# supyuxiang/Inference-Time-Scaling-for-Diffusion-Models-beyond-Scaling-Denoising-Steps

Measured on NVIDIA B200. Metric: candidate images/sec (T=1000 NFE, verifier incl.), higher is better.
Workload: dtype bf16/fp16 operands, fp32 accumulate

## Files before the change

inference-time-scaling-for-diffusion-models-beyond-scaling-denoising-steps_b200/csrc/conv_persist_sm100.cu:

```cuda
#include "tapgemm.cuh"
#include "sm100_ptx.cuh"

namespace its {

constexpr int P_THREADS = 352;
constexpr int P_EPI_THREADS = 256;
constexpr int PANEL_COLS = 64;
constexpr int PANEL_BYTES = BM * PANEL_COLS * 2;

template <int BN, int STAGES, int MT, int KS, bool TM = false>
struct PersistSmem {
  static constexpr int B_BYTES = BN * BK * 2;
  static constexpr int STAGE_BYTES = KS * (MT * A_BYTES + B_BYTES);
  static constexpr int STAGING_OFF = STAGES * STAGE_BYTES;
  static constexpr int RED_OFF = STAGING_OFF + 2 * PANEL_BYTES;
  static constexpr int RED_BYTES = 2 * 8 * 16 * 8;
  static constexpr int BAR_OFF = RED_OFF + RED_BYTES;
  static constexpr int NBARS = 2 * STAGES + 8;
  static constexpr int TOTAL = BAR_OFF + NBARS * 8 + 16;
  static constexpr int TMEM_COLS = (2 * MT * BN <= 128) ? 128 : (2 * MT * BN <= 256) ? 256 : 512;
  static_assert(2 * MT * BN <= 512, "TMEM holds two accumulator sets");
  static_assert(!TM || (BN == 128 && MT == 2 && KS == 1), "transposed mode: 128 channels x 256 pixels");
};

struct TileCoord {
  int phase, n0, tx, ty, tb;
};

__device__ __forceinline__ TileCoord decode_tile(const TapGemmParams& p, int tile, int tiles_m, int tiles_n,
                                                  int bn, int mt_per_tile) {
  TileCoord c;
  const int tpp = tiles_m * tiles_n;
  c.phase = tile / tpp;
  const int r = tile - c.phase * tpp;
  const int nt = r / tiles_m;
  const int mt = r - nt * tiles_m;
  c.n0 = nt * bn;
  const int ty_tiles = p.tiles_y / mt_per_tile;
  c.tx = mt % p.tiles_x;
  c.ty = (mt / p.tiles_x) % ty_tiles;
  c.tb = mt / (p.tiles_x * ty_tiles);
  return c;
}

struct WorkItem {
  int tile, split;
};
__device__ __forceinline__ WorkItem decode_item(int w, int total_tiles, int S) {
  WorkItem it;
  if (S == 1) {
    it.tile = w;
    it.split = 0;
  } else {
    const int npart = total_tiles * (S - 1);
    if (w < npart) {
      it.tile = w / (S - 1);
      it.split = w - it.tile * (S - 1);
    } else {
      it.tile = w - npart;
      it.split = S - 1;
    }
  }
  return it;
}

template <bool H>
__device__ __forceinline__ void tm_stage_column(const uint32_t* v, float alpha, float bvs, uint32_t sbuf_addr, int half,
                                                uint32_t chunk, uint32_t col_byte, float& s, float& qq) {
#pragma unroll
  for (int i = 0; i < 64; ++i) {
    const uint32_t prow = (uint32_t)(half * 64 + i);
    const float f = fmaf(__uint_as_float(v[i]), alpha, bvs);
    unsigned short hb;
    float r;
    if (H) {
      const __half hh = __float2half_rn(f);
      r = __half2float(hh);
      hb = __half_as_ushort(hh);
    } else {
      const __nv_bfloat16 h = __float2bfloat16_rn(f);
      r = __bfloat162float(h);
      hb = __bfloat16_as_ushort(h);
    }
    s += r;
    qq = fmaf(r, r, qq);
// ... 14 lines not shown
    const uint32_t dst = row_addr + (uint32_t)(((half * 4 + g) ^ (row & 7)) << 4);
    const uint4 u = *reinterpret_cast<const uint4*>(&pk);
    asm volatile("st.shared.v4.b32 [%0], {%1, %2, %3, %4};" ::"r"(dst), "r"(u.x), "r"(u.y), "r"(u.z), "r"(u.w)
                 : "memory");
  }
}

template <bool H>
__device__ __forceinline__ void column_pair_sums(uint32_t sbuf_addr, int r8, int cp, float& s, float& qq) {
#pragma unroll
  for (int i = 0; i < 16; ++i) {
    const int r = r8 * 16 + i;
    const uint32_t a = sbuf_addr + (uint32_t)r * 128u + (uint32_t)((((cp >> 2) ^ (r & 7)) << 4) | ((cp & 3) << 2));
    uint32_t wv;
    asm volatile("ld.shared.b32 %0, [%1];" : "=r"(wv) : "r"(a));
    float x0, x1;
    decode2_fmt(wv, H, x0, x1);
    s += x0 + x1;
    qq = fmaf(x0, x0, qq);
    qq = fmaf(x1, x1, qq);
  }
}

__device__ __forceinline__ void gn_peer_rendezvous(unsigned* counter, unsigned peers) {
  __threadfence();
  const unsigned old = atomicAdd(counter, 1u);
  const unsigned target = (old / peers + 1u) * peers;
  if (old + 1u != target) {
    unsigned cur = old;
    for (uint32_t spin = 0; spin < (1u << 24); ++spin) {
      asm volatile("ld.acquire.gpu.global.u32 %0, [%1];" : "=r"(cur) : "l"(counter) : "memory");
      if ((int)(cur - target) >= 0) break;
      __nanosleep(20);
    }
    if ((int)(cur - target) < 0) __trap();
  }
  __threadfence();
}

__device__ __forceinline__ void gn_tile_stats(float2* table, const float2* stats, int et, int pairs, int ngt, int g0,
                                              int img0, int n_img, int parts, int nchunk, int cg4, double n, float eps) {
  int T = P_EPI_THREADS / pairs;
  if (T > 32) T = 32;
  const int pr = et / T, l = et - pr * T;
  const int il = pr / ngt, gl = pr - il * ngt;
  const long long bi = img0 + il;
  const bool active = pr < pairs && bi < n_img;
  double s = 0.0, q = 0.0;
  if (active) {
    const float2* base = stats + bi * parts * nchunk + (g0 + gl) * cg4;
    const int E = parts * cg4;
// ... 92 lines not shown
    tma_prefetch_desc(&tmB);
    tma_prefetch_desc(&tmOut);
    if constexpr (GN) tma_prefetch_desc(&tmGn);
  }
  if (warp == 1) {
    asm volatile("tcgen05.alloc.cta_group::1.sync.aligned.shared::cta.b32 [%0], %1;" ::"r"(smem_u32(tmem_slot)),
                 "r"((uint32_t)L::TMEM_COLS)
                 : "memory");
    asm volatile("tcgen05.relinquish_alloc_permit.cta_group::1.sync.aligned;" ::: "memory");
  }
  tcgen05_fence_before();
  __syncthreads();
  tcgen05_fence_after();
  const uint32_t tmem_base = *tmem_slot;
  asm volatile("griddepcontrol.launch_dependents;" ::: "memory");
  if (warp != 0) asm volatile("griddepcontrol.wait;" ::: "memory");
  if (dbg != nullptr && threadIdx.x == 0) dbg[2] = clock64();

  if (warp == 0) {
    uint32_t npre = 0;
    auto produce = [&](const bool pre) {
      uint32_t it = 0;
      for (int w = blockIdx.x; w < total_items; w += gridDim.x) {
        const WorkItem wi = decode_item(w, total_tiles, S);
        const TileCoord c = decode_tile(p, wi.tile, tiles_m, tiles_n, BN, MT);
        const DevPhase& ph = p.phase[c.phase];
        const int kb0 = (ph.nkb * wi.split) / S, kb1 = (ph.nkb * (wi.split + 1)) / S;
        const int wb = (p.w_batch_stride != 0) ? c.tb * p.bb : 0;
        int g = 0;
        for (int t = 0; t < ph.ntaps && g < kb1; ++t) {
          const int si = ph.src[t];
          const DevSrc& s = p.src[si];
          const int ncb = s.C / BK;
          if (g + ncb <= kb0) { g += ncb; continue; }
          const CUtensorMap* tm = (si == 0) ? &tmA0 : (si == 1) ? &tmA1 : &tmA2;
          const int cx = c.tx * p.bw * s.stride + ph.dx[t];
          const int cy = c.ty * (p.bh * MT) * s.stride + ph.dy[t];
          const int cb_img = s.bcast ? 0 : c.tb * p.bb;
          for (int cb = 0; cb < ncb; cb += KS, g += KS) {
            if (g < kb0 || g >= kb1) continue;
            if (pre && it >= (uint32_t)STAGES) { npre = it; return; }
            const uint32_t stage = it % STAGES;
            const uint32_t parity = (it / STAGES) & 1u;
            if (!pre) mbar_wait(&empty_bar[stage], parity ^ 1u);
            if (elect_one_sync()) {
              uint8_t* a_dst = smem + stage * L::STAGE_BYTES;
              uint8_t* b_dst = a_dst + KS * MT * A_BYTES;
// ... 2 lines not shown
#pragma unroll
                for (int u = 0; u < KS; ++u)
                  tma_load_3d(b_dst + u * L::B_BYTES, &tmB, &full_bar[stage], ph.w_k0 + (g + u) * BK, c.n0, wb);
              }
              if (!pre) {
#pragma unroll
                for (int u = 0; u < KS; ++u)
                  tma_load_4d(a_dst + u * MT * A_BYTES, tm, &full_bar[stage], (cb + u) * BK, cx, cy, cb_img);
              }
            }
            __syncwarp();
            ++it;
          }
        }
      }
      if (pre) npre = it;
    };
    if (p.w_batch_stride == 0) produce(true);
    asm volatile("griddepcontrol.wait;" ::: "memory");
    produce(false);
  } else if (warp == 1) {
    uint32_t it = 0, j = 0;
    for (int w = blockIdx.x; w < total_items; w += gridDim.x, ++j) {
      const WorkItem wi = decode_item(w, total_tiles, S);
      const DevPhase& ph = p.phase[wi.tile / (tiles_m * tiles_n)];
      const int nkb_phase = ph.nkb;
      const int kb0 = (nkb_phase * wi.split) / S;
      const int nkb = (nkb_phase * (wi.split + 1)) / S - kb0;
      const uint32_t idesc_a = make_idesc(BN, ph.fp16_first != 0), idesc_b = make_idesc(BN, ph.fp16_first == 0);
      const int ksw = ph.kb_switch - kb0;
      const uint32_t buf = j & 1u;
      mbar_wait(&tempty_bar[buf], ((j >> 1) & 1u) ^ 1u);
      tcgen05_fence_after();
      const uint32_t d_tmem = tmem_base + buf * (MT * BN);
      for (int kb = 0; kb < nkb; kb += KS, ++it) {
        const uint32_t stage = it % STAGES;
        const uint32_t parity = (it / STAGES) & 1u;
        const uint32_t idesc = kb < ksw ? idesc_a : idesc_b;
        mbar_wait(&full_bar[stage], parity);
        tcgen05_fence_after();
        if (elect_one_sync()) {
          const uint32_t a_addr = smem_u32(smem + stage * L::STAGE_BYTES);
          const uint32_t b_addr = a_addr + KS * MT * A_BYTES;
          if constexpr (TM) {
            const uint64_t wdesc = make_smem_desc(b_addr), xdesc = make_smem_desc(a_addr);
            const uint32_t idesc_t = (idesc & ~(0x3Fu << 17)) | ((uint32_t)(256 >> 3) << 17);
#pragma unroll
// ... 16 lines not shown
          if (kb + KS >= nkb) umma_commit(&tfull_bar[buf]);
        }
        __syncwarp();
      }
    }
  } else if (warp < 10) {
    const int q = warp & 3;
    const int half = (warp - 2) >> 2;
    const int row = q * 32 + lane;
    const int et = (warp - 2) * 32 + lane;
    const int rpi = BM / p.bb;
    const int rb = row / rpi;
    const int nsb_img = 8 / p.bb;
    const int tiles_img = p.tiles_x * p.tiles_y;
    const int cp = et & 31, r8 = et >> 5;
    const int st_ch = et & 15, st_ib = et >> 4;
    float2* prev_dst = nullptr;
    constexpr bool fuse_gn = GN;
    const bool gn_silu = p.gn_silu != 0;
    const int gn_cg = fuse_gn ? p.Cout / p.gn_groups : 4;
    const float2* stats2 = reinterpret_cast<const float2*>(p.stats);
    uint32_t j = 0, pc = 0;
    for (int w = blockIdx.x; w < total_items; w += gridDim.x, ++j) {
      const WorkItem wi = decode_item(w, total_tiles, S);
      const TileCoord c = decode_tile(p, wi.tile, tiles_m, tiles_n, BN, MT);
      const uint32_t buf = j & 1u;
      constexpr int NPANEL = BN / PANEL_COLS;
      if (S > 1) {
        int* flags = reinterpret_cast<int*>(p.ws);
        float* parts = p.ws + p.ws_flag_words;
        if (wi.split < S - 1) {
          mbar_wait(&tfull_bar[buf], (j >> 1) & 1u);
          tcgen05_fence_after();
          float* wsrow = parts + ((long long)(wi.tile * (S - 1) + wi.split) * BM + row) * BN + half * 32;
#pragma unroll 1
          for (int pn = 0; pn < NPANEL; ++pn) {
            uint32_t v[32];
            tmem_ld32_nowait(tmem_base + ((uint32_t)(q * 32) << 16) + buf * (MT * BN) +
                                 (uint32_t)(pn * PANEL_COLS + half * 32), v);
            tmem_wait_ld();
            float4* dst = reinterpret_cast<float4*>(wsrow + pn * PANEL_COLS);
#pragma unroll
            for (int i = 0; i < 8; ++i)
              __stcg(dst + i, make_float4(__uint_as_float(v[4 * i]), __uint_as_float(v[4 * i + 1]),
                                          __uint_as_float(v[4 * i + 2]), __uint_as_float(v[4 * i + 3])));
          }
          tcgen05_fence_before();
          mbar_arrive(&tempty_bar[buf]);
          __threadfence();
          named_bar_sync(1, P_EPI_THREADS);
          if (et == 0) {
            int* f = flags + wi.tile * (S - 1) + wi.split;
            asm volatile("st.release.gpu.global.s32 [%0], %1;" ::"l"(f), "r"(1) : "memory");
          }
          continue;
        }
        if (et == 0) {
          for (int sp = 0; sp < S - 1; ++sp) {
            int* f = flags + wi.tile * (S - 1) + sp;
            int seen = 0;
            for (uint32_t spin = 0; spin < (1u << 24); ++spin) {
              asm volatile("ld.acquire.gpu.global.s32 %0, [%1];" : "=r"(seen) : "l"(f) : "memory");
              if (seen != 0) break;
              __nanosleep(64);
            }
            if (seen == 0) __trap();
            *f = 0;
          }
        }
        named_bar_sync(1, P_EPI_THREADS);
      }
      if constexpr (TM) {
        const int cglob = c.n0 + row;
        const int bimg = c.tb;
        float bvs = p.bias ? __ldg(p.bias + cglob) : 0.f;
        if (p.vec) bvs += __ldg(p.vec + (long long)bimg * p.vec_stride + cglob);
        if (p.vec2) bvs += __ldg(p.vec2 + (long long)bimg * p.vec2_stride + cglob);
        mbar_wait(&tfull_bar[buf], (j >> 1) & 1u);
        tcgen05_fence_after();
        if (dbg != nullptr && et == 0 && j < 8) dbg[8 + j] = clock64();
        const int pn = q >> 1;
        const uint32_t cc = (uint32_t)((q & 1) * 32 + lane);
#pragma unroll 1
        for (int m = 0; m < 2; ++m) {
          const uint32_t P = pc + 2 * m + pn;
          const uint32_t sb = P & 1u;
          uint8_t* sbuf = staging + sb * PANEL_BYTES;
          uint32_t v[64];
          const uint32_t taddr = tmem_base + ((uint32_t)(q * 32) << 16) + buf * (MT * BN) +
                                 (uint32_t)(m * 128 + half * 64);
          tmem_ld32_nowait(taddr, v);
          tmem_ld32_nowait(taddr + 32, v + 32);
          mbar_wait(&pempty_bar[sb], ((P >> 1) & 1u) ^ 1u);
// ... 6 lines not shown
          const uint32_t col_byte = (cc & 7u) * 2u;
          const uint32_t chunk = cc >> 3;
          tm_stage_column<F16>(v, p.alpha, bvs, smem_u32(sbuf), half, chunk, col_byte, s, qq);
          fence_proxy_async_smem();
          mbar_arrive(&pfull_bar[sb]);
          if (p.stats != nullptr) {
            s += __shfl_xor_sync(0xffffffffu, s, 1);
            qq += __shfl_xor_sync(0xffffffffu, qq, 1);
            s += __shfl_xor_sync(0xffffffffu, s, 2);
            qq += __shfl_xor_sync(0xffffffffu, qq, 2);
            if ((lane & 3) == 0) {
              const int ty = c.ty * MT + m;
              const int part = ((c.phase * tiles_img + ty * p.tiles_x + c.tx) << 1) + half;
              reinterpret_cast<float2*>(p.stats)[((long long)bimg * p.stats_parts + part) * (p.Cout >> 2) + (cglob >> 2)] =
                  make_float2(s, qq);
            }
          }
        }
        pc += 4;
        if constexpr (GN) {
          if (p.gn_peers > 1) {
            named_bar_sync(1, P_EPI_THREADS);
            if (et == 0)
              gn_peer_rendezvous(reinterpret_cast<unsigned*>(p.gn_sync) + c.tb * tiles_n + c.n0 / BN, (unsigned)p.gn_peers);
          } else {
            __threadfence();
          }
          named_bar_sync(1, P_EPI_THREADS);
          const int ngt = BN / gn_cg, g0 = c.n0 / gn_cg;
          gn_tile_stats(red, stats2, et, ngt, ngt, g0, bimg, p.B, p.stats_parts, p.Cout >> 2, gn_cg >> 2,
                        (double)gn_cg * (double)(p.Hm * p.Wm), p.gn_eps);
          named_bar_sync(1, P_EPI_THREADS);
          const float2 mr = red[cglob / gn_cg - g0];
          const float sc = mr.y * __ldg(p.gn_gamma + cglob);
          const float gA = p.alpha * sc;
          const float gB = fmaf(bvs, sc, __ldg(p.gn_beta + cglob) - mr.x * sc);
#pragma unroll 1
          for (int m = 0; m < 2; ++m) {
            const uint32_t P = pc + 2 * m + pn;
            const uint32_t sb = P & 1u;
            uint8_t* sbuf = staging + sb * PANEL_BYTES;
            uint32_t v[64];
            const uint32_t taddr = tmem_base + ((uint32_t)(q * 32) << 16) + buf * (MT * BN) +
                                   (uint32_t)(m * 128 + half * 64);
            tmem_ld32_nowait(taddr, v);
            tmem_ld32_nowait(taddr + 32, v + 32);
            mbar_wait(&pempty_bar[sb], ((P >> 1) & 1u) ^ 1u);
            tmem_wait_ld();
            if (m == 1) {
              tcgen05_fence_before();
              mbar_arrive(&tempty_bar[buf]);
            }
            tm_stage_column_gn(v, gA, gB, gn_silu, smem_u32(sbuf), half, cc >> 3, (cc & 7u) * 2u);
            fence_proxy_async_smem();
            mbar_arrive(&pfull_bar[sb]);
          }
          pc += 4;
          named_bar_sync(1, P_EPI_THREADS);
        }
        if (dbg != nullptr && et == 0 && j < 8) dbg[24 + j] = clock64();
        continue;
      }
      int b = c.tb * p.bb + rb;
      if (b >= p.B) b = p.B - 1;
      const float* vrow = p.vec ? p.vec + (long long)b * p.vec_stride : nullptr;
      const float* vrow2 = p.vec2 ? p.vec2 + (long long)b * p.vec2_stride : nullptr;
#pragma unroll 1
      for (int pi = 0; pi < MT * NPANEL; ++pi, ++pc) {
        const int m = pi / NPANEL, pn = pi - m * NPANEL;
        const int n = c.n0 + pn * PANEL_COLS;
        const int nc = n + half * 32;
        const int ty = c.ty * MT + m;
        const uint32_t sb = pc & 1u, spar = (pc >> 1) & 1u;
        uint8_t* sbuf = staging + sb * PANEL_BYTES;
        float bv[32];
#pragma unroll
        for (int i = 0; i < 32; ++i) bv[i] = 0.f;
        if (p.bias) {
#pragma unroll
          for (int i = 0; i < 8; ++i) {
            const float4 t4 = __ldg(reinterpret_cast<const float4*>(p.bias + nc) + i);
            bv[4 * i] = t4.x; bv[4 * i + 1] = t4.y; bv[4 * i + 2] = t4.z; bv[4 * i + 3] = t4.w;
          }
        }
        if (vrow) {
#pragma unroll
          for (int i = 0; i < 8; ++i) {
            const float4 t4 = __ldg(reinterpret_cast<const float4*>(vrow + nc) + i);
            bv[4 * i] += t4.x; bv[4 * i + 1] += t4.y; bv[4 * i + 2] += t4.z; bv[4 * i + 3] += t4.w;
          }
        }
        if (vrow2) {
#pragma unroll
          for (int i = 0; i < 8; ++i) {
            const float4 t4 = __ldg(reinterpret_cast<const float4*>(vrow2 + nc) + i);
            bv[4 * i] += t4.x; bv[4 * i + 1] += t4.y; bv[4 * i + 2] += t4.z; bv[4 * i + 3] += t4.w;
          }
        }
        if (pi == 0) {
          mbar_wait(&tfull_bar[buf], (j >> 1) & 1u);
          tcgen05_fence_after();
          if (dbg != nullptr && et == 0 && j < 8) dbg[8 + j] = clock64();
        }
        uint32_t v[32];
        const uint32_t taddr = tmem_base + ((uint32_t)(q * 32) << 16) + buf * (MT * BN) +
                               (uint32_t)(m * BN + pn * PANEL_COLS + half * 32);
        tmem_ld32_nowait(taddr, v);
        mbar_wait(&pempty_bar[sb], spar ^ 1u);
        tmem_wait_ld();
        if (pi == MT * NPANEL - 1 && !fuse_gn) {
          tcgen05_fence_before();
          mbar_arrive(&tempty_bar[buf]);
        }
        if (S > 1) {
          const float* prow = p.ws + p.ws_flag_words +
                              ((long long)(wi.tile * (S - 1)) * BM + row) * BN + pn * PANEL_COLS + half * 32;
          float acc[32];
          for (int sp = 0; sp < S - 1; ++sp) {
            const float4* src = reinterpret_cast<const float4*>(prow + (long long)sp * BM * BN);
#pragma unroll
            for (int i = 0; i < 8; ++i) {
              const float4 t4 = __ldcg(src + i);
              if (sp == 0) {
                acc[4 * i] = t4.x; acc[4 * i + 1] = t4.y; acc[4 * i + 2] = t4.z; acc[4 * i + 3] = t4.w;
              } else {
                acc[4 * i] += t4.x; acc[4 * i + 1] += t4.y; acc[4 * i + 2] += t4.z; acc[4 * i + 3] += t4.w;
              }
            }
          }
#pragma unroll
          for (int i = 0; i < 32; ++i) v[i] = __float_as_uint(acc[i] + __uint_as_float(v[i]));
        }
        const uint32_t row_addr = smem_u32(sbuf) + (uint32_t)row * 128u;
        stage_row32<F16>(v, p.alpha, bv, row_addr, half, row);
        fence_proxy_async_smem();
        mbar_arrive(&pfull_bar[sb]);
        if (p.stats != nullptr && p.bb > 8) {
          mbar_wait(&pfull_bar[sb], spar);
          for (int idx = et; idx < p.bb * 16; idx += P_EPI_THREADS) {
            const int ib = idx >> 4, ch = idx & 15;
            const int bi = c.tb * p.bb + ib;
            if (bi >= p.B) continue;
            float s = 0.f, qq = 0.f;
            for (int r = ib * rpi; r < (ib + 1) * rpi; ++r) {
              const uint32_t a = smem_u32(sbuf) + (uint32_t)r * 128u +
                                 (uint32_t)((((ch >> 1) ^ (r & 7)) << 4) | ((ch & 1) << 3));
              uint32_t w0, w1;
              asm volatile("ld.shared.v2.b32 {%0, %1}, [%2];" : "=r"(w0), "=r"(w1) : "r"(a));
              float x0, x1, x2, x3;
              decode2_fmt(w0, F16, x0, x1);
              decode2_fmt(w1, F16, x2, x3);
              s += (x0 + x1) + (x2 + x3);
              qq = fmaf(x0, x0, qq); qq = fmaf(x1, x1, qq); qq = fmaf(x2, x2, qq); qq = fmaf(x3, x3, qq);
            }
// ... 22 lines not shown
          if (et < 16 * p.bb && bi < p.B) {
            const int part = (p.bb == 1) ? c.phase * tiles_img + ty * p.tiles_x + c.tx : c.phase;
            prev_dst = reinterpret_cast<float2*>(p.stats) +
                       ((long long)bi * p.stats_parts + part) * (p.Cout >> 2) + (n >> 2) + st_ch;
          }
        }
      }
      if constexpr (GN) {
        named_bar_sync(1, P_EPI_THREADS);
        if (prev_dst != nullptr) {
          const float2* rd = red + ((pc + 1) & 1u) * 128;
          float S1 = 0.f, Q1 = 0.f;
          for (int k = 0; k < nsb_img; ++k) {
            const float2 t2 = rd[(st_ib * nsb_img + k) * 16 + st_ch];
            S1 += t2.x;
            Q1 += t2.y;
          }
          *prev_dst = make_float2(S1, Q1);
          prev_dst = nullptr;
        }
        if (p.gn_peers > 1) {
          named_bar_sync(1, P_EPI_THREADS);
          if (et == 0)
            gn_peer_rendezvous(reinterpret_cast<unsigned*>(p.gn_sync) + c.tb * tiles_n + c.n0 / BN, (unsigned)p.gn_peers);
        } else {
          __threadfence();
        }
        named_bar_sync(1, P_EPI_THREADS);
        const int NG = BN / gn_cg, g0 = c.n0 / gn_cg;
        gn_tile_stats(red, stats2, et, p.bb * NG, NG, g0, c.tb * p.bb, p.B, p.stats_parts, p.Cout >> 2, gn_cg >> 2,
                      (double)gn_cg * (double)(p.Hm * p.Wm), p.gn_eps);
        named_bar_sync(1, P_EPI_THREADS);
#pragma unroll 1
        for (int pi = 0; pi < MT * NPANEL; ++pi, ++pc) {
          const int m = pi / NPANEL, pn = pi - m * NPANEL;
          const int nc = c.n0 + pn * PANEL_COLS + half * 32;
          const uint32_t sb = pc & 1u, spar = (pc >> 1) & 1u;
          uint8_t* sbuf = staging + sb * PANEL_BYTES;
          uint32_t v[32];
          const uint32_t taddr = tmem_base + ((uint32_t)(q * 32) << 16) + buf * (MT * BN) +
                                 (uint32_t)(m * BN + pn * PANEL_COLS + half * 32);
          tmem_ld32_nowait(taddr, v);
          mbar_wait(&pempty_bar[sb], spar ^ 1u);
          tmem_wait_ld();
          if (pi == MT * NPANEL - 1) {
            tcgen05_fence_before();
            mbar_arrive(&tempty_bar[buf]);
          }
          const float* prow = p.ws + p.ws_flag_words +
                              ((long long)(wi.tile * (S - 1)) * BM + row) * BN + pn * PANEL_COLS + half * 32;
          const uint32_t row_addr = smem_u32(sbuf) + (uint32_t)row * 128u;
#pragma unroll
          for (int k8 = 0; k8 < 4; ++k8) {
            float f[8];
#pragma unroll
            for (int h4 = 0; h4 < 2; ++h4) {
              const int k = 2 * k8 + h4;
              float x[4] = {__uint_as_float(v[4 * k]), __uint_as_float(v[4 * k + 1]), __uint_as_float(v[4 * k + 2]),
                            __uint_as_float(v[4 * k + 3])};
              if (S > 1) {
                float4 acc = __ldcg(reinterpret_cast<const float4*>(prow) + k);
                for (int sp = 1; sp < S - 1; ++sp) {
                  const float4 t4 = __ldcg(reinterpret_cast<const float4*>(prow + (long long)sp * BM * BN) + k);
                  acc.x += t4.x; acc.y += t4.y; acc.z += t4.z; acc.w += t4.w;
                }
                x[0] = acc.x + x[0]; x[1] = acc.y + x[1]; x[2] = acc.z + x[2]; x[3] = acc.w + x[3];
              }
              float add[4] = {0.f, 0.f, 0.f, 0.f};
              if (p.bias) {
                const float4 t4 = __ldg(reinterpret_cast<const float4*>(p.bias + nc) + k);
                add[0] = t4.x; add[1] = t4.y; add[2] = t4.z; add[3] = t4.w;
              }
              if (vrow) {
                const float4 t4 = __ldg(reinterpret_cast<const float4*>(vrow + nc) + k);
                add[0] += t4.x; add[1] += t4.y; add[2] += t4.z; add[3] += t4.w;
              }
              if (vrow2) {
                const float4 t4 = __ldg(reinterpret_cast<const float4*>(vrow2 + nc) + k);
                add[0] += t4.x; add[1] += t4.y; add[2] += t4.z; add[3] += t4.w;
              }
              const float2 mr = red[rb * NG + (nc + 4 * k) / gn_cg - g0];
              const float4 g4 = __ldg(reinterpret_cast<const float4*>(p.gn_gamma + nc) + k);
              const float4 b4 = __ldg(reinterpret_cast<const float4*>(p.gn_beta + nc) + k);
              const float gg[4] = {g4.x, g4.y, g4.z, g4.w}, bt[4] = {b4.x, b4.y, b4.z, b4.w};
#pragma unroll
              for (int jj = 0; jj < 4; ++jj) {
                const float sc = mr.y * gg[jj];
                f[4 * h4 + jj] = gn_act(x[jj], p.alpha * sc, fmaf(add[jj], sc, bt[jj] - mr.x * sc), gn_silu);
              }
            }
// ... 8 lines not shown
        }
        named_bar_sync(1, P_EPI_THREADS);
      }
      if (dbg != nullptr && et == 0 && j < 8) dbg[24 + j] = clock64();
    }
    if (p.stats != nullptr) {
      named_bar_sync(1, P_EPI_THREADS);
      if (prev_dst != nullptr) {
        const float2* rd = red + ((pc + 1) & 1u) * 128;
        float S = 0.f, Q = 0.f;
        for (int k = 0; k < nsb_img; ++k) {
          const float2 t2 = rd[(st_ib * nsb_img + k) * 16 + st_ch];
          S += t2.x;
          Q += t2.y;
        }
        *prev_dst = make_float2(S, Q);
      }
    }
  } else if (warp == 10) {
    if (lane == 0) {
      uint32_t pc = 0;
      constexpr int NPANEL = BN / PANEL_COLS;
      for (int w = blockIdx.x; w < total_items; w += gridDim.x) {
        const WorkItem wi = decode_item(w, total_tiles, S);
        if (wi.split < S - 1) continue;
        const TileCoord c = decode_tile(p, wi.tile, tiles_m, tiles_n, BN, MT);
        const DevPhase& ph = p.phase[c.phase];
        constexpr int npass = GN ? 2 : 1;
        for (int pass = 0; pass < npass; ++pass) {
          for (int pi = 0; pi < MT * NPANEL; ++pi, ++pc) {
            const int m = pi / NPANEL, pn = pi - m * NPANEL;
            const int n = c.n0 + pn * PANEL_COLS;
            const int ty = c.ty * MT + m;
            const uint32_t sb = pc & 1u, spar = (pc >> 1) & 1u;
            const uint8_t* sbuf = staging + sb * PANEL_BYTES;
            mbar_wait(&pfull_bar[sb], spar);
            if (pass == 0 && p.gn_only) {
              mbar_arrive(&pempty_bar[sb]);
              continue;
            }
            if (pass == 1)
              tma_store_3d(&tmGn, sbuf, n, c.tx * p.bw, c.tb * p.bb * p.Hm + ty * p.bh);
            else if (p.out_scale == 1)
              tma_store_3d(&tmOut, sbuf, n, c.tx * p.bw, c.tb * p.bb * p.Hm + ty * p.bh);
            else
              tma_store_5d(&tmOut, sbuf, n, ph.px, c.tx * p.bw, ph.py, c.tb * p.bb * p.Hm + ty * p.bh);
            bulk_commit_group();
            bulk_wait_group_read<0>();
            mbar_arrive(&pempty_bar[sb]);
          }
        }
      }
      bulk_wait_group<0>();
// ... 60 lines not shown
bool tapgemm_persist_eligible(const its_conv_desc* d, const TapGemmParams& p) {
  if (p.out_fp32 || p.out_nchw || p.res != nullptr) return false;
  if (p.w_batch_stride != 0 && (p.bb != 1 || p.splits > 1)) return false;
  if (p.Cout % 64 != 0 || p.out_c_pitch % 8 != 0) return false;
  const int bn = persist_bn(d, p);
  if (!(bn == 64 || bn == 128 || bn == 192 || bn == 256) || p.Cout % bn != 0) return false;
  if (p.bw * p.bh * p.bb != BM || p.Wm % p.bw != 0 || p.Hm % p.bh != 0) return false;
  if (p.bb > 1 && p.bh != p.Hm) return false;
  return true;
}

template <int BN, int STAGES, int MT, int KS, bool TM, bool F16, bool GN>
static int launch_persist_fmt(const TapGemmParams& p, const CUtensorMap* tmA, const CUtensorMap& tmB,
                              const CUtensorMap& tmOut, const CUtensorMap& tmGn, cudaStream_t stream) {
  using L = PersistSmem<BN, STAGES, MT, KS, TM>;
  static_assert(L::TOTAL <= 227 * 1024, "shared memory budget");
  auto kern = tapgemm_persist_kernel<BN, STAGES, MT, KS, TM, F16, GN>;
  static PerDeviceBytes configured;
  if (configured.need(L::TOTAL))
    ITS_CHECK_CUDA(cudaFuncSetAttribute(kern, cudaFuncAttributeMaxDynamicSharedMemorySize, L::TOTAL));
  const int tiles = p.tiles_x * (p.tiles_y / MT) * p.tiles_b * (p.Cout / BN) * p.nphases * p.splits;
  const int sms = device_sm_count();
  cudaLaunchConfig_t cfg = {};
  cfg.gridDim = dim3(tiles < sms ? tiles : sms, 1, 1);
  cfg.blockDim = dim3(P_THREADS, 1, 1);
  cfg.dynamicSmemBytes = L::TOTAL;
  cfg.stream = stream;
  cudaLaunchAttribute attr[1];
  attr[0].id = cudaLaunchAttributeProgrammaticStreamSerialization;
  attr[0].val.programmaticStreamSerializationAllowed = 1;
  cfg.attrs = attr;
  cfg.numAttrs = pdl_enabled(1) ? 1 : 0;
  ITS_CHECK_CUDA(cudaLaunchKernelEx(&cfg, kern, p, tmA[0], tmA[1], tmA[2], tmB, tmOut, tmGn));
  return ITS_OK;
}

template <int BN, int STAGES, int MT, int KS, bool TM = false>
static int launch_persist(const TapGemmParams& p, const CUtensorMap* tmA, const CUtensorMap& tmB,
                          const CUtensorMap& tmOut, const CUtensorMap& tmGn, cudaStream_t stream) {
  if (p.gn_out != nullptr) {
    if (p.out_fp16) return launch_persist_fmt<BN, STAGES, MT, KS, TM, true, true>(p, tmA, tmB, tmOut, tmGn, stream);
    return launch_persist_fmt<BN, STAGES, MT, KS, TM, false, true>(p, tmA, tmB, tmOut, tmGn, stream);
  }
  if (p.out_fp16) return launch_persist_fmt<BN, STAGES, MT, KS, TM, true, false>(p, tmA, tmB, tmOut, tmGn, stream);
  return launch_persist_fmt<BN, STAGES, MT, KS, TM, false, false>(p, tmA, tmB, tmOut, tmGn, stream);
}

int tapgemm_launch_persist(const its_conv_desc* d, const TapGemmParams& p, cudaStream_t stream) {
  const int bn = persist_bn(d, p);
  ITS_REQUIRE(tapgemm_persist_eligible(d, p), "its_conv_igemm: layer not eligible for the persistent kernel");
  ITS_REQUIRE(p.w_pitch % 8 == 0 && (reinterpret_cast<uintptr_t>(p.w) & 15) == 0, "its_conv_igemm: weight alignment");
  ITS_REQUIRE((reinterpret_cast<uintptr_t>(p.out) & 15) == 0, "its_conv_igemm: output pointer alignment");
  if (p.stats != nullptr)
    ITS_REQUIRE(p.stats_parts == tapgemm_stats_parts(d, p), "its_conv_igemm: stats_parts=%d, the tiling writes %d",
                p.stats_parts, tapgemm_stats_parts(d, p));
  const PersistCfg cfg = persist_cfg(d, p);
  const int mt = cfg.mt;
  TapGemmParams pp = p;
  if (p.splits > 1) {
    const long long tiles = (long long)p.tiles_x * p.tiles_y * p.tiles_b * (p.Cout / bn) * p.nphases;
    const long long nflag = ((tiles * (p.splits - 1) + 63) / 64) * 64;
    const long long need = nflag + tiles * (p.splits - 1) * BM * bn;
    ITS_REQUIRE(d->ws != nullptr && d->ws_elems >= need,
                "its_conv_igemm: persistent split-K workspace has %lld floats, %lld needed (must be zero-initialised)",
                (long long)d->ws_elems, need);
    for (int f = 0; f < p.nphases; ++f)
      ITS_REQUIRE(p.splits <= p.phase[f].nkb, "its_conv_igemm: splits=%d exceeds the %d k-blocks of phase %d", p.splits, p.phase[f].nkb, f);
    pp.ws_flag_words = (int)nflag;
  }
  if (p.gn_out != nullptr) {
    const int words = tapgemm_gn_sync_words(d, p);
    ITS_REQUIRE(words >= 0, "its_conv_igemm: this layer's GroupNorm cannot be fused into its epilogue "
                "(its_conv_gn_sync_words() < 0): Cout=%d groups=%d bn=%d", p.Cout, p.gn_groups, bn);
    ITS_REQUIRE(p.stats != nullptr, "its_conv_igemm: the fused GroupNorm epilogue needs the statistics array");
    ITS_REQUIRE(p.gn_gamma != nullptr && p.gn_beta != nullptr, "its_conv_igemm: gn_gamma / gn_beta");
    ITS_REQUIRE(words == 0 || p.gn_sync != nullptr, "its_conv_igemm: gn_sync needs %d zero-initialised ints", words);
    ITS_REQUIRE(p.gn_c_pitch >= p.Cout && p.gn_c_pitch % 8 == 0 && (reinterpret_cast<uintptr_t>(p.gn_out) & 15) == 0,
                "its_conv_igemm: gn_out pitch / alignment");
    pp.gn_sync_words = words;
    pp.gn_peers = p.tiles_x * (p.tiles_y / mt);
  }
  CUtensorMap tmA[ITS_MAX_SRC], tmB, tmOut, tmGn;
  int rc = tapgemm_encode_operand_maps(p, bn, tmA, &tmB, mt);
  if (rc != ITS_OK) return rc;
  const cuuint64_t pitch_b = (cuuint64_t)p.out_c_pitch * 2;
  if (p.out_scale == 1) {
    const cuuint64_t dims[3] = {(cuuint64_t)p.Cout, (cuuint64_t)p.Wm, (cuuint64_t)p.B * p.Hm};
    const cuuint64_t strides[2] = {pitch_b, pitch_b * p.Wout};
    const cuuint32_t box[3] = {(cuuint32_t)PANEL_COLS, (cuuint32_t)p.bw, (cuuint32_t)(p.bh * p.bb)};
    const cuuint32_t estr[3] = {1, 1, 1};
    rc = encode_bf16_map(&tmOut, 3, p.out, dims, strides, box, estr, "output");
// ... 43 lines not shown
```

inference-time-scaling-for-diffusion-models-beyond-scaling-denoising-steps_b200/csrc/tapgemm.cuh:

```cuda
#pragma once
#include "its_common.cuh"
#include <cuda.h>

namespace its {

struct DevSrc {
  const __nv_bfloat16* ptr;
  int c_pitch, C, H, W, stride, bcast, fp16;
};

struct DevPhase {
  int ntaps, w_k0, py, px;
  int nkb;
  int fp16_first;
  int kb_switch;
  int8_t src[ITS_MAX_TAPS], dy[ITS_MAX_TAPS], dx[ITS_MAX_TAPS];
};

struct TapGemmParams {
  DevSrc src[ITS_MAX_SRC];
  DevPhase phase[ITS_MAX_PHASES];
  int nsrc, nphases;
  int B, Hm, Wm;
  const __nv_bfloat16* w;
  int w_pitch;
  long long w_batch_stride;
  int Cout;
  void* out;
  int out_fp32, Hout, Wout, out_scale, out_c_pitch;
  const float* bias;
  const float* vec;
  int vec_stride;
  const float* vec2;
  int vec2_stride;
  const __nv_bfloat16* res;
  int res_c_pitch;
  float alpha;
  int out_nchw;
  int splits;
  float* ws;
  int ws_flag_words;
  long long* dbg;
  float* stats;
  int stats_parts;
  int out_fp16;
  int res_fp16;
  void* gn_out;
  int gn_c_pitch;
  const float* gn_gamma;
  const float* gn_beta;
  int gn_groups;
  float gn_eps;
  int gn_silu, gn_only;
  int* gn_sync;
  int gn_sync_words;
  int gn_peers;
  int bw, bh, bb, tiles_x, tiles_y, tiles_b;
};

int tapgemm_build_params(const its_conv_desc* d, TapGemmParams* p, bool need_k64);
int tapgemm_launch_ref(const TapGemmParams& p, cudaStream_t stream);
int tapgemm_launch_sm100(const its_conv_desc* d, const TapGemmParams& p, cudaStream_t stream);
bool tapgemm_persist_eligible(const its_conv_desc* d, const TapGemmParams& p);
int tapgemm_launch_persist(const its_conv_desc* d, const TapGemmParams& p, cudaStream_t stream);
// ... 11 lines not shown
```

inference-time-scaling-for-diffusion-models-beyond-scaling-denoising-steps_b200/engine.py:

```python
from __future__ import annotations

import ctypes as C
import math
from typing import List, Optional, Sequence, Tuple

import torch

from . import _lib
from ._lib import ConvDesc

BF16 = torch.bfloat16
FP16 = torch.float16
import os as _os
FP16_GN = _os.environ.get("ITS_FP16_GN", "1") != "0"


def _ptr(t: Optional[torch.Tensor]) -> Optional[int]:
    return None if t is None else t.data_ptr()


def pack_conv_weight(w: torch.Tensor) -> torch.Tensor:
    return w.detach().float().permute(0, 2, 3, 1).reshape(w.shape[0], -1)


# ... 90 lines not shown
        return tiles_m, bn

    DESIGN_BATCH = 64

    def _splits_for(self, B, Hm, Wm, cout, nphases, nkb_min, per_image_w) -> int:
        tiles_m, bn = self._tiles(self.DESIGN_BATCH, Hm, Wm, cout, per_image_w)
        ctas = tiles_m * -(-cout // bn) * nphases
        if ctas >= 96:
            return 1
        s = min(148 // ctas, nkb_min // 4, 16)
        return max(1, s)

    @staticmethod
    def _box(Hm: int, Wm: int) -> Tuple[int, int, int]:
        bw = min(Wm, 128)
        bh = min(Hm, 128 // bw)
        return bw, bh, 128 // (bw * bh)

    def _tiles_at(self, B: int, Hm: int, Wm: int) -> int:
        bw, bh, bb = self._box(Hm, Wm)
        return -(-Wm // bw) * -(-Hm // bh) * -(-B // bb)

    _T_KB = {256: 290.0, 192: 250.0, 128: 215.0, 64: 175.0}
    _T_SPLIT2 = 5000.0

    def _fusion_pays(self, Hm, Wm, cout, nkb) -> bool:
        bw, bh, bb = self._box(Hm, Wm)
        return bb == 1 and cout == 128 and Hm * Wm >= 1024 and nkb >= 36

    _SPLIT_BNS = tuple(int(x) for x in _os.environ.get("ITS_SPLIT_BNS", "64").split(","))

    def _persist_plan(self, Hm, Wm, cout, nphases, nkb, group_width: int = 0) -> Tuple[int, int]:
        bw, bh, bb = self._box(Hm, Wm)
        tiles_y = -(-Hm // bh)
        tiles_m = self._tiles_at(self.DESIGN_BATCH, Hm, Wm)
        best = None
        for bn in (256, 192, 128, 64):
            if cout % bn or (group_width and bn % group_width):
                continue
            tiles = tiles_m * (cout // bn) * nphases
            two_rows = bn <= 128 and bb == 1 and tiles_y % 2 == 0
            for S in (1, 2):
                if S > 1 and (bn not in self._SPLIT_BNS or nkb < 16 or tiles * S > self.sm_count or two_rows):
                    break
                if two_rows:
                    rounds = -(-(tiles // 2) // self.sm_count)
                    t = rounds * nkb * 410.0
                else:
                    rounds = -(-(tiles * S) // self.sm_count)
                    t = rounds * -(-nkb // S) * self._T_KB[bn]
                if S > 1:
                    t += self._T_SPLIT2
                if best is None or t < best[0] - 1e-9:
                    best = (t, bn, S)
        if best is None:
            return 0, 0
        return best[1], best[2]

    def conv(self, srcs, phases, Hm, Wm, w, cout, *, out=None, out_scale=1, bias=None, vec=None,
             vec_off=0, vec2=None, vec2_off=0, res=None, alpha=1.0, out_fp32=False, w_batch_stride=0,
             w_pitch=None, B=None, out_shape=None, out_nchw=False, want_stats=True, out_dtype=None,
             fuse_gn=None, gn_only=False) -> torch.Tensor:
        B = self.n_img if B is None else B
        d = ConvDesc()
        d.nsrc = len(srcs)
        for i, (t, c_used, c_off, stride, bcast) in enumerate(srcs):
            s = d.src[i]
            s.ptr, s.c_pitch, s.c_off, s.C = t.data_ptr(), t.shape[-1], c_off, c_used
            s.H, s.W, s.stride, s.bcast = t.shape[1], t.shape[2], stride, int(bcast)
            s.fp16 = int(t.dtype == FP16)
        d.nphases = len(phases)
        flops = 0
        for i, (taps, w_k0, py, px) in enumerate(phases):
            ph = d.phase[i]
            ph.ntaps, ph.w_k0, ph.py, ph.px = len(taps), w_k0, py, px
# ... 39 lines not shown
            bn, splits = 0, 0
            if want_fuse:
                bn, splits = self._persist_plan(Hm, Wm, cout, len(phases), nkb_plan, cout // fuse_gn[0].num_groups)
            if bn == 0:
                want_fuse = False
                bn, splits = self._persist_plan(Hm, Wm, cout, len(phases), nkb_plan)
        if persistent:
            if can_fold:
                k_used = sum(srcs[si][1] for si, _, _ in phases[0][0])
                w = torch.cat([w[:, :k_used].float(), torch.eye(cout, device=w.device)], 1)
                i = d.nsrc
                sN = d.src[i]
                sN.ptr, sN.c_pitch, sN.c_off, sN.C = res.data_ptr(), res.shape[-1], 0, cout
                sN.H, sN.W, sN.stride, sN.bcast = res.shape[1], res.shape[2], 1, 0
                sN.fp16 = int(res.dtype == FP16)
                d.nsrc = i + 1
                ph = d.phase[0]
                ph.src[ph.ntaps], ph.dy[ph.ntaps], ph.dx[ph.ntaps] = i, 0, 0
                ph.ntaps += 1
                d.w_pitch = w.shape[-1]
            d.bn = bn
            if splits > 1:
                tiles = self._tiles_at(B, Hm, Wm) * (cout // bn) * len(phases)
                nflag = -(-(tiles * (splits - 1)) // 64) * 64
                need = nflag + tiles * (splits - 1) * 128 * bn
                if self.ws_persist is None or self.ws_persist.numel() < need:
                    self.ws_persist = torch.zeros(need, dtype=torch.float32, device=self.dev)
                    self.keep.append(self.ws_persist)
                d.splits, d.ws, d.ws_elems = splits, self.ws_persist.data_ptr(), self.ws_persist.numel()
            if want_stats:
                parts = self.L.its_conv_stats_parts(C.byref(d))
                st = self._new((B, parts, cout // 4, 2), torch.float32)
                d.stats, d.stats_parts = st.data_ptr(), parts
                self.stats_of[out.data_ptr()] = (st, parts)
            if want_fuse:
                gnm, gn_silu = fuse_gn
                d.gn_groups = gnm.num_groups
                words = self.L.its_conv_gn_sync_words(C.byref(d))
                if words < 0:
                    d.gn_groups = 0
                else:
                    gn_out = self._new((B, Hout, Wout, cout), FP16)
                    gamma, beta = self._hold(gnm.weight, torch.float32), self._hold(gnm.bias, torch.float32)
                    d.gn_out, d.gn_c_pitch = gn_out.data_ptr(), cout
                    d.gn_gamma, d.gn_beta, d.gn_eps = gamma.data_ptr(), beta.data_ptr(), float(gnm.eps)
                    d.gn_silu, d.gn_only = int(gn_silu), int(bool(gn_only))
                    if words > 0:
                        sync = torch.zeros(words, dtype=torch.int32, device=self.dev)
# ... 410 lines not shown
```

Before: 36.67.

## Replace serial split-K fixup with symmetric reduce-scatter across split peers

Split-K in the persistent conv kernel used to make every non-final split write its full partial tile to a workspace and flag it, while the last split waited and summed everything. Now each split writes only the column strips owned by its peers, meets them at a counter-based rendezvous, and then reduces and runs the epilogue for its own strip, so reduction and epilogue work are spread across all splits. The planner now considers S in {2,4,8} with a byte-based exchange cost model, and the grid is rounded to a multiple of S. The risk is deadlock if split peers are not co-resident, which the grid rounding is meant to prevent. It also adds rendezvous latency on every split tile.

```diff
diff --git a/inference-time-scaling-for-diffusion-models-beyond-scaling-denoising-steps_b200/csrc/conv_persist_sm100.cu b/inference-time-scaling-for-diffusion-models-beyond-scaling-denoising-steps_b200/csrc/conv_persist_sm100.cu
--- a/inference-time-scaling-for-diffusion-models-beyond-scaling-denoising-steps_b200/csrc/conv_persist_sm100.cu
+++ b/inference-time-scaling-for-diffusion-models-beyond-scaling-denoising-steps_b200/csrc/conv_persist_sm100.cu
@@ -46,21 +46,10 @@
 struct WorkItem {
   int tile, split;
 };
-__device__ __forceinline__ WorkItem decode_item(int w, int total_tiles, int S) {
+__device__ __forceinline__ WorkItem decode_item(int w, int S) {
   WorkItem it;
-  if (S == 1) {
-    it.tile = w;
-    it.split = 0;
-  } else {
-    const int npart = total_tiles * (S - 1);
-    if (w < npart) {
-      it.tile = w / (S - 1);
-      it.split = w - it.tile * (S - 1);
-    } else {
-      it.tile = w - npart;
-      it.split = S - 1;
-    }
-  }
+  it.tile = w / S;
+  it.split = w - it.tile * S;
   return it;
 }
 
@@ -121,11 +110,11 @@
   }
 }
 
-__device__ __forceinline__ void gn_peer_rendezvous(unsigned* counter, unsigned peers) {
+__device__ __forceinline__ void peer_rendezvous(unsigned* counter, unsigned quantum, unsigned step) {
   __threadfence();
-  const unsigned old = atomicAdd(counter, 1u);
-  const unsigned target = (old / peers + 1u) * peers;
-  if (old + 1u != target) {
+  const unsigned old = atomicAdd(counter, step);
+  const unsigned target = (old / quantum + 1u) * quantum;
+  if (old + step != target) {
     unsigned cur = old;
     for (uint32_t spin = 0; spin < (1u << 24); ++spin) {
       asm volatile("ld.acquire.gpu.global.u32 %0, [%1];" : "=r"(cur) : "l"(counter) : "memory");
@@ -264,7 +253,7 @@
     auto produce = [&](const bool pre) {
       uint32_t it = 0;
       for (int w = blockIdx.x; w < total_items; w += gridDim.x) {
-        const WorkItem wi = decode_item(w, total_tiles, S);
+        const WorkItem wi = decode_item(w, S);
         const TileCoord c = decode_tile(p, wi.tile, tiles_m, tiles_n, BN, MT);
         const DevPhase& ph = p.phase[c.phase];
         const int kb0 = (ph.nkb * wi.split) / S, kb1 = (ph.nkb * (wi.split + 1)) / S;
@@ -313,7 +302,7 @@
   } else if (warp == 1) {
     uint32_t it = 0, j = 0;
     for (int w = blockIdx.x; w < total_items; w += gridDim.x, ++j) {
-      const WorkItem wi = decode_item(w, total_tiles, S);
+      const WorkItem wi = decode_item(w, S);
       const DevPhase& ph = p.phase[wi.tile / (tiles_m * tiles_n)];
       const int nkb_phase = ph.nkb;
       const int kb0 = (nkb_phase * wi.split) / S;
@@ -376,53 +365,38 @@
     const float2* stats2 = reinterpret_cast<const float2*>(p.stats);
     uint32_t j = 0, pc = 0;
     for (int w = blockIdx.x; w < total_items; w += gridDim.x, ++j) {
-      const WorkItem wi = decode_item(w, total_tiles, S);
+      const WorkItem wi = decode_item(w, S);
       const TileCoord c = decode_tile(p, wi.tile, tiles_m, tiles_n, BN, MT);
       const uint32_t buf = j & 1u;
       constexpr int NPANEL = BN / PANEL_COLS;
+      const int nps = NPANEL / S;
+      const int pi0 = (S > 1) ? wi.split * nps : 0;
+      const int pi1 = (S > 1) ? pi0 + nps : MT * NPANEL;
+      const float* xown = nullptr;
       if (S > 1) {
-        int* flags = reinterpret_cast<int*>(p.ws);
-        float* parts = p.ws + p.ws_flag_words;
-        if (wi.split < S - 1) {
-          mbar_wait(&tfull_bar[buf], (j >> 1) & 1u);
-          tcgen05_fence_after();
-          float* wsrow = parts + ((long long)(wi.tile * (S - 1) + wi.split) * BM + row) * BN + half * 32;
+        float* xbuf = p.ws + p.ws_counter_words;
+        const long long strip_elems = (long long)BM * (BN / S);
+        mbar_wait(&tfull_bar[buf], (j >> 1) & 1u);
+        tcgen05_fence_after();
 #pragma unroll 1
-          for (int pn = 0; pn < NPANEL; ++pn) {
-            uint32_t v[32];
-            tmem_ld32_nowait(tmem_base + ((uint32_t)(q * 32) << 16) + buf * (MT * BN) +
-                                 (uint32_t)(pn * PANEL_COLS + half * 32), v);
-            tmem_wait_ld();
-            float4* dst = reinterpret_cast<float4*>(wsrow + pn * PANEL_COLS);
-#pragma unroll
-            for (int i = 0; i < 8; ++i)
-              __stcg(dst + i, make_float4(__uint_as_float(v[4 * i]), __uint_as_float(v[4 * i + 1]),
-                                          __uint_as_float(v[4 * i + 2]), __uint_as_float(v[4 * i + 3])));
-          }
-          tcgen05_fence_before();
-          mbar_arrive(&tempty_bar[buf]);
-          __threadfence();
-          named_bar_sync(1, P_EPI_THREADS);
-          if (et == 0) {
-            int* f = flags + wi.tile * (S - 1) + wi.split;
-            asm volatile("st.release.gpu.global.s32 [%0], %1;" ::"l"(f), "r"(1) : "memory");
-          }
-          continue;
-        }
-        if (et == 0) {
-          for (int sp = 0; sp < S - 1; ++sp) {
-            int* f = flags + wi.tile * (S - 1) + sp;
-            int seen = 0;
-            for (uint32_t spin = 0; spin < (1u << 24); ++spin) {
-              asm volatile("ld.acquire.gpu.global.s32 %0, [%1];" : "=r"(seen) : "l"(f) : "memory");
-              if (seen != 0) break;
-              __nanosleep(64);
-            }
-            if (seen == 0) __trap();
-            *f = 0;
-          }
+        for (int pn = 0; pn < NPANEL; ++pn) {
+          const int strip = pn / nps;
+          if (strip == wi.split) continue;
+          uint32_t v[32];
+          tmem_ld32_nowait(tmem_base + ((uint32_t)(q * 32) << 16) + buf * (MT * BN) +
+                               (uint32_t)(pn * PANEL_COLS + half * 32), v);
+          tmem_wait_ld();
+          float4* dst = reinterpret_cast<float4*>(xbuf + (long long)((wi.tile * S + strip) * S + wi.split) * strip_elems) +
+                        ((pn - strip * nps) * PANEL_COLS + half * 32) / 4 * BM + row;
+#pragma unroll
+          for (int i = 0; i < 8; ++i)
+            __stcg(dst + i * BM, make_float4(__uint_as_float(v[4 * i]), __uint_as_float(v[4 * i + 1]),
+                                             __uint_as_float(v[4 * i + 2]), __uint_as_float(v[4 * i + 3])));
         }
         named_bar_sync(1, P_EPI_THREADS);
+        if (et == 0) peer_rendezvous(reinterpret_cast<unsigned*>(p.ws) + wi.tile, 8u, 8u / (unsigned)S);
+        named_bar_sync(1, P_EPI_THREADS);
+        xown = xbuf + (long long)(wi.tile * S + wi.split) * S * strip_elems + (half * 32 / 4 * BM + row) * 4;
       }
       if constexpr (TM) {
         const int cglob = c.n0 + row;
@@ -475,7 +449,7 @@
           if (p.gn_peers > 1) {
             named_bar_sync(1, P_EPI_THREADS);
             if (et == 0)
-              gn_peer_rendezvous(reinterpret_cast<unsigned*>(p.gn_sync) + c.tb * tiles_n + c.n0 / BN, (unsigned)p.gn_peers);
+              peer_rendezvous(reinterpret_cast<unsigned*>(p.gn_sync) + c.tb * tiles_n + c.n0 / BN, (unsigned)p.gn_peers, 1u);
           } else {
             __threadfence();
           }
@@ -519,7 +493,7 @@
       const float* vrow = p.vec ? p.vec + (long long)b * p.vec_stride : nullptr;
       const float* vrow2 = p.vec2 ? p.vec2 + (long long)b * p.vec2_stride : nullptr;
 #pragma unroll 1
-      for (int pi = 0; pi < MT * NPANEL; ++pi, ++pc) {
+      for (int pi = pi0; pi < pi1; ++pi, ++pc) {
         const int m = pi / NPANEL, pn = pi - m * NPANEL;
         const int n = c.n0 + pn * PANEL_COLS;
         const int nc = n + half * 32;
@@ -550,7 +524,7 @@
             bv[4 * i] += t4.x; bv[4 * i + 1] += t4.y; bv[4 * i + 2] += t4.z; bv[4 * i + 3] += t4.w;
           }
         }
-        if (pi == 0) {
+        if (S == 1 && pi == 0) {
           mbar_wait(&tfull_bar[buf], (j >> 1) & 1u);
           tcgen05_fence_after();
           if (dbg != nullptr && et == 0 && j < 8) dbg[8 + j] = clock64();
@@ -561,28 +535,31 @@
         tmem_ld32_nowait(taddr, v);
         mbar_wait(&pempty_bar[sb], spar ^ 1u);
         tmem_wait_ld();
-        if (pi == MT * NPANEL - 1 && !fuse_gn) {
+        if (pi == pi1 - 1 && !fuse_gn) {
           tcgen05_fence_before();
           mbar_arrive(&tempty_bar[buf]);
         }
         if (S > 1) {
-          const float* prow = p.ws + p.ws_flag_words +
-                              ((long long)(wi.tile * (S - 1)) * BM + row) * BN + pn * PANEL_COLS + half * 32;
+          const float* src = xown + (pi - pi0) * PANEL_COLS * BM;
           float acc[32];
-          for (int sp = 0; sp < S - 1; ++sp) {
-            const float4* src = reinterpret_cast<const float4*>(prow + (long long)sp * BM * BN);
-#pragma unroll
-            for (int i = 0; i < 8; ++i) {
-              const float4 t4 = __ldcg(src + i);
-              if (sp == 0) {
-                acc[4 * i] = t4.x; acc[4 * i + 1] = t4.y; acc[4 * i + 2] = t4.z; acc[4 * i + 3] = t4.w;
-              } else {
-                acc[4 * i] += t4.x; acc[4 * i + 1] += t4.y; acc[4 * i + 2] += t4.z; acc[4 * i + 3] += t4.w;
+          for (int jj = 0; jj < S; ++jj) {
+            float x[32];
+            if (jj == wi.split) {
+#pragma unroll
+              for (int i = 0; i < 32; ++i) x[i] = __uint_as_float(v[i]);
+            } else {
+              const float4* s4 = reinterpret_cast<const float4*>(src + (long long)jj * BM * (BN / S));
+#pragma unroll
+              for (int i = 0; i < 8; ++i) {
+                const float4 t4 = __ldcg(s4 + i * BM);
+                x[4 * i] = t4.x; x[4 * i + 1] = t4.y; x[4 * i + 2] = t4.z; x[4 * i + 3] = t4.w;
               }
             }
-          }
-#pragma unroll
-          for (int i = 0; i < 32; ++i) v[i] = __float_as_uint(acc[i] + __uint_as_float(v[i]));
+#pragma unroll
+            for (int i = 0; i < 32; ++i) acc[i] = (jj == 0) ? x[i] : acc[i] + x[i];
+          }
+#pragma unroll
+          for (int i = 0; i < 32; ++i) v[i] = __float_as_uint(acc[i]);
         }
         const uint32_t row_addr = smem_u32(sbuf) + (uint32_t)row * 128u;
         stage_row32<F16>(v, p.alpha, bv, row_addr, half, row);
@@ -651,7 +628,7 @@
         if (p.gn_peers > 1) {
           named_bar_sync(1, P_EPI_THREADS);
           if (et == 0)
-            gn_peer_rendezvous(reinterpret_cast<unsigned*>(p.gn_sync) + c.tb * tiles_n + c.n0 / BN, (unsigned)p.gn_peers);
+            peer_rendezvous(reinterpret_cast<unsigned*>(p.gn_sync) + c.tb * tiles_n + c.n0 / BN, (unsigned)p.gn_peers, 1u);
         } else {
           __threadfence();
         }
@@ -676,8 +653,6 @@
             tcgen05_fence_before();
             mbar_arrive(&tempty_bar[buf]);
           }
-          const float* prow = p.ws + p.ws_flag_words +
-                              ((long long)(wi.tile * (S - 1)) * BM + row) * BN + pn * PANEL_COLS + half * 32;
           const uint32_t row_addr = smem_u32(sbuf) + (uint32_t)row * 128u;
 #pragma unroll
           for (int k8 = 0; k8 < 4; ++k8) {
@@ -687,14 +662,6 @@
               const int k = 2 * k8 + h4;
               float x[4] = {__uint_as_float(v[4 * k]), __uint_as_float(v[4 * k + 1]), __uint_as_float(v[4 * k + 2]),
                             __uint_as_float(v[4 * k + 3])};
-              if (S > 1) {
-                float4 acc = __ldcg(reinterpret_cast<const float4*>(prow) + k);
-                for (int sp = 1; sp < S - 1; ++sp) {
-                  const float4 t4 = __ldcg(reinterpret_cast<const float4*>(prow + (long long)sp * BM * BN) + k);
-                  acc.x += t4.x; acc.y += t4.y; acc.z += t4.z; acc.w += t4.w;
-                }
-                x[0] = acc.x + x[0]; x[1] = acc.y + x[1]; x[2] = acc.z + x[2]; x[3] = acc.w + x[3];
-              }
               float add[4] = {0.f, 0.f, 0.f, 0.f};
               if (p.bias) {
                 const float4 t4 = __ldg(reinterpret_cast<const float4*>(p.bias + nc) + k);
@@ -749,13 +716,15 @@
       uint32_t pc = 0;
       constexpr int NPANEL = BN / PANEL_COLS;
       for (int w = blockIdx.x; w < total_items; w += gridDim.x) {
-        const WorkItem wi = decode_item(w, total_tiles, S);
-        if (wi.split < S - 1) continue;
+        const WorkItem wi = decode_item(w, S);
         const TileCoord c = decode_tile(p, wi.tile, tiles_m, tiles_n, BN, MT);
         const DevPhase& ph = p.phase[c.phase];
+        const int nps = NPANEL / S;
+        const int pi0 = (S > 1) ? wi.split * nps : 0;
+        const int pi1 = (S > 1) ? pi0 + nps : MT * NPANEL;
         constexpr int npass = GN ? 2 : 1;
         for (int pass = 0; pass < npass; ++pass) {
-          for (int pi = 0; pi < MT * NPANEL; ++pi, ++pc) {
+          for (int pi = pi0; pi < pi1; ++pi, ++pc) {
             const int m = pi / NPANEL, pn = pi - m * NPANEL;
             const int n = c.n0 + pn * PANEL_COLS;
             const int ty = c.ty * MT + m;
@@ -862,7 +831,8 @@
   const int tiles = p.tiles_x * (p.tiles_y / MT) * p.tiles_b * (p.Cout / BN) * p.nphases * p.splits;
   const int sms = device_sm_count();
   cudaLaunchConfig_t cfg = {};
-  cfg.gridDim = dim3(tiles < sms ? tiles : sms, 1, 1);
+  const int grid = tiles < sms ? tiles : (sms / p.splits) * p.splits;
+  cfg.gridDim = dim3(grid, 1, 1);
   cfg.blockDim = dim3(P_THREADS, 1, 1);
   cfg.dynamicSmemBytes = L::TOTAL;
   cfg.stream = stream;
@@ -898,15 +868,22 @@
   const int mt = cfg.mt;
   TapGemmParams pp = p;
   if (p.splits > 1) {
+    const int S = p.splits;
+    ITS_REQUIRE(S == 2 || S == 4 || S == 8, "its_conv_igemm: persistent split-K needs splits in {2, 4, 8}, got %d", S);
+    ITS_REQUIRE(bn % (S * PANEL_COLS) == 0, "its_conv_igemm: split-K strips of bn=%d / splits=%d columns are not whole "
+                "64-column panels", bn, S);
+    ITS_REQUIRE(mt == 1 && !cfg.tm, "its_conv_igemm: split-K takes one row box per tile");
+    ITS_REQUIRE(p.gn_out == nullptr, "its_conv_igemm: the fused GroupNorm epilogue does not combine with split-K");
+    for (int f = 0; f < p.nphases; ++f)
+      ITS_REQUIRE(p.phase[f].nkb % S == 0, "its_conv_igemm: splits=%d does not divide the %d k-blocks of phase %d",
+                  S, p.phase[f].nkb, f);
     const long long tiles = (long long)p.tiles_x * p.tiles_y * p.tiles_b * (p.Cout / bn) * p.nphases;
-    const long long nflag = ((tiles * (p.splits - 1) + 63) / 64) * 64;
-    const long long need = nflag + tiles * (p.splits - 1) * BM * bn;
+    const long long ncount = ((tiles + 63) / 64) * 64;
+    const long long need = ncount + tiles * S * BM * bn;
     ITS_REQUIRE(d->ws != nullptr && d->ws_elems >= need,
-                "its_conv_igemm: persistent split-K workspace has %lld floats, %lld needed (must be zero-initialised)",
+                "its_conv_igemm: persistent split-K workspace has %lld floats, %lld needed (counters zero-initialised once)",
                 (long long)d->ws_elems, need);
-    for (int f = 0; f < p.nphases; ++f)
-      ITS_REQUIRE(p.splits <= p.phase[f].nkb, "its_conv_igemm: splits=%d exceeds the %d k-blocks of phase %d", p.splits, p.phase[f].nkb, f);
-    pp.ws_flag_words = (int)nflag;
+    pp.ws_counter_words = (int)ncount;
   }
   if (p.gn_out != nullptr) {
     const int words = tapgemm_gn_sync_words(d, p);
diff --git a/inference-time-scaling-for-diffusion-models-beyond-scaling-denoising-steps_b200/csrc/tapgemm.cuh b/inference-time-scaling-for-diffusion-models-beyond-scaling-denoising-steps_b200/csrc/tapgemm.cuh
--- a/inference-time-scaling-for-diffusion-models-beyond-scaling-denoising-steps_b200/csrc/tapgemm.cuh
+++ b/inference-time-scaling-for-diffusion-models-beyond-scaling-denoising-steps_b200/csrc/tapgemm.cuh
@@ -39,7 +39,7 @@
   int out_nchw;
   int splits;
   float* ws;
-  int ws_flag_words;
+  int ws_counter_words;
   long long* dbg;
   float* stats;
   int stats_parts;
diff --git a/inference-time-scaling-for-diffusion-models-beyond-scaling-denoising-steps_b200/engine.py b/inference-time-scaling-for-diffusion-models-beyond-scaling-denoising-steps_b200/engine.py
--- a/inference-time-scaling-for-diffusion-models-beyond-scaling-denoising-steps_b200/engine.py
+++ b/inference-time-scaling-for-diffusion-models-beyond-scaling-denoising-steps_b200/engine.py
@@ -136,13 +136,15 @@
         return -(-Wm // bw) * -(-Hm // bh) * -(-B // bb)
 
     _T_KB = {256: 290.0, 192: 250.0, 128: 215.0, 64: 175.0}
-    _T_SPLIT2 = 5000.0
+    _T_RDV = 2560.0
+    _T_XCHG_BYTE = 0.025
+
+    def _split_cost(self, bn: int, S: int) -> float:
+        return self._T_RDV + self._T_XCHG_BYTE * 2.0 * (S - 1) / S * 128 * bn * 4
 
     def _fusion_pays(self, Hm, Wm, cout, nkb) -> bool:
         bw, bh, bb = self._box(Hm, Wm)
         return bb == 1 and cout == 128 and Hm * Wm >= 1024 and nkb >= 36
-
-    _SPLIT_BNS = tuple(int(x) for x in _os.environ.get("ITS_SPLIT_BNS", "64").split(","))
 
     def _persist_plan(self, Hm, Wm, cout, nphases, nkb, group_width: int = 0) -> Tuple[int, int]:
         bw, bh, bb = self._box(Hm, Wm)
@@ -154,17 +156,15 @@
                 continue
             tiles = tiles_m * (cout // bn) * nphases
             two_rows = bn <= 128 and bb == 1 and tiles_y % 2 == 0
-            for S in (1, 2):
-                if S > 1 and (bn not in self._SPLIT_BNS or nkb < 16 or tiles * S > self.sm_count or two_rows):
-                    break
+            for S in (1, 2, 4, 8):
+                if S > 1 and (group_width or two_rows or bn % (64 * S) or nkb % S or nkb // S < 4):
+                    continue
                 if two_rows:
                     rounds = -(-(tiles // 2) // self.sm_count)
                     t = rounds * nkb * 410.0
                 else:
-                    rounds = -(-(tiles * S) // self.sm_count)
-                    t = rounds * -(-nkb // S) * self._T_KB[bn]
-                if S > 1:
-                    t += self._T_SPLIT2
+                    rounds = -(-(tiles * S) // (self.sm_count // S * S))
+                    t = rounds * ((nkb // S) * self._T_KB[bn] + (self._split_cost(bn, S) if S > 1 else 0.0))
                 if best is None or t < best[0] - 1e-9:
                     best = (t, bn, S)
         if best is None:
@@ -250,8 +250,7 @@
             d.bn = bn
             if splits > 1:
                 tiles = self._tiles_at(B, Hm, Wm) * (cout // bn) * len(phases)
-                nflag = -(-(tiles * (splits - 1)) // 64) * 64
-                need = nflag + tiles * (splits - 1) * 128 * bn
+                need = -(-tiles // 64) * 64 + tiles * splits * 128 * bn
                 if self.ws_persist is None or self.ws_persist.numel() < need:
                     self.ws_persist = torch.zeros(need, dtype=torch.float32, device=self.dev)
                     self.keep.append(self.ws_persist)
```

After: 37.51, median of 6. 2.3% higher.
